# THU-luvision/TextureFusion

Measured on AMD Instinct MI355X. Metric: RGB-D frames/s (TSDF integrate + atlas update: prepare->integrate->finalize, UpdateMeshes, GeneratePatches + UpdateAtlas over the frame's dirty chunks), higher is better.
Workload: dtype f32

## Files before the change

texturefusion_amd/csrc/tf_group.hip:

```cpp
#include <hip/hip_runtime.h>
#include <stdlib.h>

#include <type_traits>

#include "tf_device.h"
#include "tf_devfn.h"
#include "tf_host_math.h"
#include "tf_voxel_math.h"

#pragma clang fp contract(off)

namespace tf {

constexpr int kGroupMax = 6;
struct GroupArgs {
  const float* depth[kGroupMax];
  const float4* pre[kGroupMax];
  const float* cen[kGroupMax];
  int n;
};

struct GroupPoses {
  Pose P[kGroupMax];
};
// ... 83 lines not shown
          __builtin_amdgcn_make_buffer_rsrc((void*)key.img.depth, 0, W * H * 4, 0x00020000);
      const __amdgpu_buffer_rsrc_t rs_rgba =
          __builtin_amdgcn_make_buffer_rsrc((void*)key.img.rgba, 0, W * H * 4, 0x00020000);
      const __amdgpu_buffer_rsrc_t rs_C =
          __builtin_amdgcn_make_buffer_rsrc((void*)(v.color + (size_t)slot * kChunkVoxels), 0, 4096, 0x00020000);
      const __amdgpu_buffer_rsrc_t rs_qual =
          __builtin_amdgcn_make_buffer_rsrc((void*)key.img.quality, 0, QUAL ? W * H * 4 : 0, 0x00020000);
      const float khalf = kc.res * 0.5f;
      const float fx = (float)(lane & 7), fy = (float)vy;
      float qx[3], qy[3];
#pragma unroll
      for (int a = 0; a < 3; ++a) { qx[a] = key.P.p[a] * fx; qy[a] = key.P.p[4 + a] * fy; }
      auto cen = [&](const int a, const int j) -> float {
        const float q2 = key.P.p[8 + a] * (float)j;
        const float s12 = qy[a] + q2;
        const float d = qx[a] + s12;
        return d * kc.res + khalf;
      };
      int off_d[8];
      unsigned long long vm[8];
      uint32_t R = 64, oob_bits = 0;
      int oob_any = 0;
      auto geometry = [&](auto safe_tag) {
        constexpr bool SAFE = decltype(safe_tag)::value;
#pragma unroll
        for (int j = 0; j < 8; ++j) {
          const f32x2 pxy = o01 + (f32x2){cen(0, j), cen(1, j)};
          const float pzv = o2 + cen(2, j);
          f32x2 q;
          if (SAFE) {
            q = div2_by(pxy, recip_refined(pzv));
          } else {
            q.x = pxy.x / pzv;
            q.y = pxy.y / pzv;
          }
          const f32x2 uw = q * fxy + cxy;
          const int X = SAFE ? cvt_rne_hw(uw.x) : cvt_sat_rne(uw.x);
          const int Y = SAFE ? cvt_rne_hw(uw.y) : cvt_sat_rne(uw.y);
          const bool valid = ((unsigned)(X - 1) < (unsigned)(W - 2)) && ((unsigned)(Y - 1) < (unsigned)(H - 2));
          vm[j] = ballot(valid);
          int od = (__mul24(Y, W) + X) * 4;
          asm volatile("" : "+v"(od));
          off_d[j] = valid ? od : kOOB;
          oob_bits |= (((unsigned)X > (unsigned)(W - 1)) || ((unsigned)Y > (unsigned)(H - 1))) ? (1u << j) : 0u;
        }
      };
      if (div_safe) geometry(std::true_type{});
      else geometry(std::false_type{});
      unsigned long long all_valid = ~0ull;
#pragma unroll
      for (int j = 0; j < 8; ++j) all_valid &= vm[j];
      if (all_valid != ~0ull) {
#pragma unroll
        for (int j = 0; j < 8; ++j) {
          if (R == 64u) {
            const unsigned long long dead = nonzero_bytes(vm[j]) ^ 0x0101010101010101ull;
            if (dead) R = (uint32_t)(j * 8) + ((uint32_t)__builtin_ctzll(dead) >> 3);
          }
          const bool live_lane = (uint32_t)(j * 8 + vy) < R;
          oob_any |= (live_lane && ((oob_bits >> j) & 1u)) ? 1 : 0;
          off_d[j] = live_lane ? off_d[j] : kOOB;
        }
      }
      float dep[8];
#pragma unroll
      for (int j = 0; j < 8; ++j)
        dep[j] = __uint_as_float(__builtin_amdgcn_raw_buffer_load_b32(rs_depth, off_d[j], 0, 0));
#pragma unroll
      for (int j = 0; j < 8; ++j) {
        if ((uint32_t)(j * 8) >= R) break;
        const float d = dep[j];
        const float sd = d - (o2 + cen(2, j));
        const bool act = (uint32_t)(j * 8 + vy) < R;
        const bool dv = (d > cam.nearP) && (cam.farP > d);
        const bool inside = (sd > kc.lower) && (upper > sd);
        const bool F = act && dv && inside;
        const float nw = F ? wD : 0.0f;
        const bool rf_l = row_any(ballot(F));
        key_rows_t += (uint32_t)__popcll(ballot(rf_l)) >> 3;
        if (rf_l) {
          const float ts = __uint_as_float(t[j].x), tw = __uint_as_float(t[j].y);
          const float num = ts * tw + sd * nw;
          const float den = (tw + nw) + kc.sigma;
          const float ns = num / den;
          const float nwt = tw + nw;
          const bool keep = nwt > 0.5f;
          t[j].x = __float_as_uint(keep ? ns : 999.0f);
          t[j].y = __float_as_uint(keep ? nwt : 0.0f);
          dirty_rows |= 1u << j;
        }
      }
      uint32_t lanes_c = 0;
      float qsum_rows = 0.0f;
      const bool some_oob = all_valid != ~0ull;
#pragma unroll
      for (int h = 0; h < 2; ++h) {
        int off_c[4], off_i[4];
        unsigned long long any_c = 0ull;
        unsigned long long mo[QUAL ? 4 : 1];
        unsigned long long any_o = 0ull;
        if (QUAL) {
#pragma unroll
          for (int jj = 0; jj < 4; ++jj) {
            const int j = h * 4 + jj;
            mo[jj] = some_oob ? ballot(((uint32_t)(j * 8 + vy) < R) && ((oob_bits >> j) & 1u)) : 0ull;
            any_o |= mo[jj];
          }
        }
#pragma unroll
        for (int jj = 0; jj < 4; ++jj) {
          const int j = h * 4 + jj;
          const float sd = dep[j] - (o2 + cen(2, j));
          const bool upd = (off_d[j] != kOOB) && (fabsf(sd) < kc.thrCol);
          off_i[jj] = upd ? off_d[j] : kOOB;
          const bool ru_l = row_any(ballot(upd));
          const unsigned long long ru = ballot(ru_l);
          off_c[jj] = ru_l ? (j * 64 + lane) * 8 : kOOB;
          lanes_c += (uint32_t)__popcll(ru);
          any_c |= ru;
        }
        if (any_c == 0ull) {
          if (QUAL && any_o) {
#pragma unroll
            for (int jj = 0; jj < 4; ++jj)
              if (mo[jj]) qsum_rows = kc.qoob;
          }
          continue;
        }
        u32x2 c[4];
        uint32_t in[4];
        float qv[QUAL ? 4 : 1];
#pragma unroll
        for (int jj = 0; jj < 4; ++jj) {
          c[jj] = __builtin_amdgcn_raw_buffer_load_b64(rs_C, off_c[jj], 0, 0);
          in[jj] = __builtin_amdgcn_raw_buffer_load_b32(rs_rgba, off_i[jj], 0, 0);
          if (QUAL) qv[jj] = __uint_as_float(__builtin_amdgcn_raw_buffer_load_b32(rs_qual, off_i[jj], 0, 0));
        }
#pragma unroll
        for (int jj = 0; jj < 4; ++jj) {
          const uint32_t p_rg = __builtin_amdgcn_perm(0u, in[jj], 0x0c010c00u);
          const uint32_t p_ba = __builtin_amdgcn_perm(0u, in[jj], 0x0c030c02u);
          const uint32_t w_rg = c[jj].x, w_ba = c[jj].y;
          const u16x2 in_rg = __builtin_bit_cast(u16x2, p_rg), in_ba = __builtin_bit_cast(u16x2, p_ba);
          u16x2 c_rg = __builtin_bit_cast(u16x2, w_rg), c_ba = __builtin_bit_cast(u16x2, w_ba);
          if (FLAG) {
            c_rg += in_rg;
            c_ba += in_ba;
            const bool halve = (int)__builtin_bit_cast(uint32_t, c_ba) >= (121 << 16);
            const u16x2 h_rg = c_rg >> (unsigned short)2, h_ba = c_ba >> (unsigned short)2;
            c_rg = halve ? h_rg : c_rg;
            c_ba = halve ? h_ba : c_ba;
          } else {
            c_rg -= in_rg;
            c_ba -= in_ba;
          }
          c[jj].x = __builtin_bit_cast(uint32_t, c_rg);
          c[jj].y = __builtin_bit_cast(uint32_t, c_ba);
          __builtin_amdgcn_raw_buffer_store_b64(c[jj], rs_C, off_c[jj], 0, 0);
        }
        if (QUAL) {
          const int rowshift = lane & 56;
#pragma unroll
          for (int jj = 0; jj < 4; ++jj) {
            const int j = h * 4 + jj;
            const unsigned long long mu = ballot(off_i[jj] != kOOB);
            if ((mu | mo[jj]) == 0ull) continue;
            float rowsum = 0.0f;
// ... 15 lines not shown
      const float qsum = QUAL ? qsum_rows : ((ballot(oob_any != 0) != 0ull) ? kc.qoob : 0.0f);
      if (lane == 0) {
        L.list_quality[e] = qsum;
        if (obs_kf >= 0 && qsum > 0.0f && key_rows_t != 0u) {
          const uint32_t at = obs_find(v, obs_pack(slot, obs_kf), true);
          if (at != kInvalidSlot) v.obs_q[at] = qsum;
        }
      }
    }
    for (int f = 0; f < ga.n; ++f) {
      const float4 r0 = ga.pre[f][4 * e], r1 = ga.pre[f][4 * e + 1];
      const float o0 = r0.x, o1 = r0.y, o2 = r0.z, pbx = r0.w, pby = r1.x;
      const f32x2 o01 = {o0, o1};
      const float wD = FLAG ? pbx : -pbx;
      const float upper = pby;
      const float band = 32.0f * kc.res;
      const bool div_safe = (fabsf(o2) > band) && (fabsf(o2) < 1048576.0f) && (fabsf(o0) < 1048576.0f) &&
                            (fabsf(o1) < 1048576.0f) && (kc.res > 1e-6f) && (kc.res < 16.0f);
      const __amdgpu_buffer_rsrc_t rs_depth =
          __builtin_amdgcn_make_buffer_rsrc((void*)ga.depth[f], 0, W * H * 4, 0x00020000);
      int off_d[8];
      unsigned long long vm[8];
      uint32_t R = 64;
      auto geometry = [&](auto safe_tag) {
        constexpr bool SAFE = decltype(safe_tag)::value;
#pragma unroll
        for (int j = 0; j < 8; ++j) {
          const int k = j * 64 + lane;
          const f32x2 pxy = o01 + (f32x2){cenT[f][0][k], cenT[f][1][k]};
          const float pzv = o2 + cenT[f][2][k];
          f32x2 q;
          if (SAFE) {
            q = div2_by(pxy, recip_refined(pzv));
          } else {
            q.x = pxy.x / pzv;
            q.y = pxy.y / pzv;
          }
          const f32x2 uw = q * fxy + cxy;
          const int X = SAFE ? cvt_rne_hw(uw.x) : cvt_sat_rne(uw.x);
          const int Y = SAFE ? cvt_rne_hw(uw.y) : cvt_sat_rne(uw.y);
          const bool valid = ((unsigned)(X - 1) < (unsigned)(W - 2)) && ((unsigned)(Y - 1) < (unsigned)(H - 2));
          vm[j] = ballot(valid);
          int od = (__mul24(Y, W) + X) * 4;
          asm volatile("" : "+v"(od));
          off_d[j] = valid ? od : kOOB;
        }
      };
      if (div_safe) geometry(std::true_type{});
      else geometry(std::false_type{});
      unsigned long long all_valid = ~0ull;
#pragma unroll
      for (int j = 0; j < 8; ++j) all_valid &= vm[j];
      if (all_valid != ~0ull) {
#pragma unroll
        for (int j = 0; j < 8; ++j) {
          if (R == 64u) {
            const unsigned long long dead = nonzero_bytes(vm[j]) ^ 0x0101010101010101ull;
            if (dead) R = (uint32_t)(j * 8) + ((uint32_t)__builtin_ctzll(dead) >> 3);
          }
          const bool live_lane = (uint32_t)(j * 8 + vy) < R;
          off_d[j] = live_lane ? off_d[j] : kOOB;
        }
      }
      float dep[8];
#pragma unroll
      for (int j = 0; j < 8; ++j)
        dep[j] = __uint_as_float(__builtin_amdgcn_raw_buffer_load_b32(rs_depth, off_d[j], 0, 0));
#pragma unroll
      for (int j = 0; j < 8; ++j) {
        if ((uint32_t)(j * 8) >= R) break;
        const float d = dep[j];
        const float sd = d - (o2 + cenT[f][2][j * 64 + lane]);
        const bool act = (uint32_t)(j * 8 + vy) < R;
        const bool dv = (d > cam.nearP) && (cam.farP > d);
        const bool inside = (sd > kc.lower) && (upper > sd);
        const bool F = act && dv && inside;
        const float nw = F ? wD : 0.0f;
        const bool rf_l = row_any(ballot(F));
        rows_total += (uint32_t)__popcll(ballot(rf_l)) >> 3;
        if (rf_l) {
          const float ts = __uint_as_float(t[j].x), tw = __uint_as_float(t[j].y);
          const float num = ts * tw + sd * nw;
          const float den = (tw + nw) + kc.sigma;
          const float ns = num / den;
          const float nwt = tw + nw;
          const bool keep = nwt > 0.5f;
          t[j].x = __float_as_uint(keep ? ns : 999.0f);
          t[j].y = __float_as_uint(keep ? nwt : 0.0f);
          dirty_rows |= 1u << j;
        }
      }
    }
    uint32_t word = 0;
#pragma unroll
    for (int j = 0; j < 8; ++j) {
      const bool wr = ((dirty_rows >> j) & 1u) != 0;
      __builtin_amdgcn_raw_buffer_store_b64(t[j], rs_T, wr ? (j * 64 + lane) * 8 : kOOB, 0, 0);
      if (wr) word |= chunk_summary_bits(__uint_as_float(t[j].x), __uint_as_float(t[j].y), (uint32_t)(j * 64 + lane));
    }
    word = wave_or(word);
    if (lane == 0 && word) atomicOr(&v.summ[slot], word);
    const bool updated = (rows_total | key_rows_t) != 0;
    if (updated && lane == 0) {
      L.list_needs[e] = 1;
      if (part_band(v, id.x, id.y, id.z)) mark_touched(v, L.list_ent[e]);
    }
    const uint32_t rows_key = KEY ? (key_rows_c << 8) : (fin ? (uint32_t)L.list_rows[e] : 0u);
    if (lane == 0) L.list_rows[e] = (uint16_t)(rows_total + key_rows_t < 255u ? rows_total + key_rows_t : 255u);
    if (fin) {
      const bool isnew = L.list_new[e] != 0;
      if (updated || L.list_needs[e]) {
        if (lane == 0) {
          v.mark_epoch[slot] = fin_epoch + 1u;
          if (isnew && !part_band(v, id.x, id.y, id.z)) v.hent[L.list_ent[e]].alive = 1u;
        }
        if (claim_par >= 0) claim_dirty7(v, id, slot, L.list_ent[e], lane, claim_stamp, claim_par);
      } else if (isnew) {
        const uint32_t ent = L.list_ent[e];
        if (rows_key >> 8) {
          uint4* c4 = reinterpret_cast<uint4*>(v.color + (size_t)slot * kChunkVoxels);
#pragma unroll
          for (int k = 0; k < 4; ++k) c4[k * 64 + lane] = make_uint4(0, 0, 0, 0);
        }
        if (v.hent[ent].alive) {
          const uint32_t ds = v.summ[slot];
          if (ds != 0u) {
            const uint32_t f999 = __float_as_uint(999.0f);
            uint4* t4 = reinterpret_cast<uint4*>(v.tsdf + (size_t)slot * kChunkVoxels);
#pragma unroll
            for (int k = 0; k < 4; ++k) t4[k * 64 + lane] = make_uint4(f999, 0u, f999, 0u);
          }
          if (lane == 0) {
            v.hent[ent].alive = 0;
            if (ds != 0u) {
              v.summ[slot] = 0u;
              MeshRec* r = &v.mesh_rec[slot];
              if (r->state & kMsInMap) { r->state = 0u; r->nv = 0; r->nt = 0; }
            }
          }
        }
        if (lane == 0) v.erase_epoch[slot] = fin_epoch + 1u;
      }
    }
  }
}


void launch_pre_frames(const VolumeDev& v, const Pose& keyframe, int n, const float* poses12, float4* pre_scratch,
                       float* cen_scratch, const Integ& ig, float res, const Cam& cam, hipStream_t s, int acquire,
                       uint32_t* clear_word) {
  const IntegrateConsts kc = make_integrate_consts(cam.cxi, cam.cyi, res, 1);
  GroupPoses gp = {};
  for (int f = 0; f < n; ++f)
    for (int q = 0; q < 12; ++q) gp.P[f].p[q] = poses12[12 * f + q];
  hipLaunchKernelGGL(k_pre_group, dim3(128, n + 1 + (acquire ? 1 : 0)), dim3(256), 0, s, v, gp, ig, res, kc.resDiag, pre_scratch,
                     cen_scratch, keyframe, 1, acquire, clear_word);
}

void launch_integrate_group(const VolumeDev& v, int n, const float* const* d_depth, const float* poses12, float4* pre_scratch,
                            float* cen_scratch, const Cam& cam, const Integ& ig, float res, int flag, hipStream_t s, bool have_pre,
                            int32_t obs_kf, int fin, uint32_t fin_epoch, int claim_par, uint32_t claim_stamp,
                            const FrameImages* key_img, const Pose* key_pose) {
  IntegrateConsts kc = make_integrate_consts(cam.cxi, cam.cyi, res, flag);
  GroupArgs ga = {};
  GroupPoses gp = {};
  ga.n = n;
  for (int f = 0; f < n; ++f) {
// ... 20 lines not shown
```

texturefusion_amd/csrc/tf_kernels.hip:

```cpp
#include <stdlib.h>

#include <atomic>
#include "tf_device.h"
#include "tf_devfn.h"
#include "tf_host_math.h"
#include "tf_patch_body.h"
#include "tf_voxel_math.h"

#pragma clang fp contract(off)
#ifndef TF_KA_GP
#define TF_KA_GP 2
#endif


namespace tf {

__global__ void k_reset_ctl(FrameCtl* ctl, VolCtl* vctl) {
  if (blockIdx.x == 0 && threadIdx.x == 0) {
    for (int a = 0; a < 3; ++a) {
      ctl->bbox_key[a] = f2key(1e8f);
      ctl->bbox_key[3 + a] = f2key(-1e8f);
      ctl->min_id[a] = ctl->max_id[a] = ctl->dims[a] = 0;
    }
    ctl->n_coarse = 0;
// ... 395 lines not shown
        int4 id;
        id.x = sx + ((step == 4) ? (lane >> 4) : 0);
        id.y = sy + ((step == 4) ? ((lane >> 2) & 3) : 0);
        id.z = sz + ((step == 4) ? (lane & 3) : 0);
        id.w = 0;
        if (pos < v.max_list) L.list_id[pos] = id;
      }
    }
    if (tile == n_tiles - 1u && threadIdx.x == 0) finish(tile_base + agg);
    __syncthreads();
  }
}
void launch_scan(const VolumeDev& v, int step, hipStream_t s) {
  static std::atomic<uint32_t> g_stamp{0};
  uint32_t stamp;
  do { stamp = (g_stamp.fetch_add(1u) + 1u) & 0x3FFFFFFFu; } while (stamp == 0u);
  hipLaunchKernelGGL(k_scan, dim3(256), dim3(256), 0, s, v, step, stamp);
}

__global__ __launch_bounds__(256) void k_acquire(VolumeDev v) {
  const SelBuf& L = v.sel;
  const uint32_t n = L.ctl->n_list;
  for (uint32_t e = blockIdx.x * 256 + threadIdx.x; e < n; e += gridDim.x * 256) {
    const int4 id = L.list_id[e];
    bool is_new = false;
    uint32_t ent = 0;
    const uint32_t slot = chunk_acquire(v, id, &is_new, &ent);
    L.list_slot[e] = slot;
    L.list_ent[e] = ent;
    L.list_new[e] = is_new ? 1 : 0;
    L.list_needs[e] = 0;
  }
}
void launch_acquire(const VolumeDev& v, hipStream_t s) {
  hipLaunchKernelGGL(k_acquire, dim3(512), dim3(256), 0, s, v);
}

__global__ __launch_bounds__(256) void k_pre(VolumeDev v, Pose P, Integ ig, float res, float resDiag, float4* out_pre,
                                             float* out_cen) {
  const SelBuf& L = v.sel;
  float4* pre = out_pre ? out_pre : L.list_pre;
  if (blockIdx.x == 0) centroid_table(P.p, res, out_cen ? out_cen : L.cen);
  const uint32_t n = L.ctl->n_list <= v.max_list ? L.ctl->n_list : 0u;
  for (uint32_t e = blockIdx.x * 256 + threadIdx.x; e < n; e += gridDim.x * 256) {
    const int4 id = L.list_id[e];
    const ChunkPre cp = chunk_pre(id, P.p, ig, res, resDiag);
    pre[4 * e] = make_float4(cp.a.x, cp.a.y, cp.a.z, cp.b.x);
    pre[4 * e + 1] = make_float4(cp.b.y, __int_as_float(id.x), __int_as_float(id.y), __int_as_float(id.z));
  }
}

__global__ __launch_bounds__(256) void k_lookup(VolumeDev v, uint32_t n) {
  const SelBuf& L = v.sel;
  const uint32_t i = blockIdx.x * 256 + threadIdx.x;
  if (i >= n) return;
  const int4 id = L.list_id[i];
  const uint32_t ent = hash_find(v, pack_id(id.x, id.y, id.z));
  uint32_t slot = kInvalidSlot;
  if (ent != kInvalidSlot && v.hent[ent].alive) slot = v.hent[ent].slot;
  if (slot == kInvalidSlot) atomicOr(&v.vctl->status, kStMissing);
  L.list_slot[i] = slot;
  L.list_ent[i] = (ent == kInvalidSlot) ? 0u : ent;
}
void launch_lookup(const VolumeDev& v, uint32_t n, hipStream_t s) {
  if (!n) return;
  hipLaunchKernelGGL(k_lookup, dim3((n + 255) / 256), dim3(256), 0, s, v, n);
}

#ifndef TF_KF_WAVES
#define TF_KF_WAVES 7
#endif
#ifndef TF_KFP_EXTRA
#define TF_KFP_EXTRA 1
#endif
#ifndef TF_KFP_WAVES
#define TF_KFP_WAVES 7
#endif

typedef uint32_t u32x4 __attribute__((ext_vector_type(4)));
typedef const __attribute__((address_space(4))) u32x4* const_u32x4_ptr;
typedef uint32_t u32x8 __attribute__((ext_vector_type(8)));
typedef const __attribute__((address_space(4))) u32x8* const_u32x8_ptr;

template <bool COLOR, bool QUALITY, bool FUSED, bool FLAG, int GP, bool TL = false>
__device__ __forceinline__ void integrate_body(const VolumeDev& v, const FrameImages& img, const Cam& cam,
                                               const IntegrateConsts& kc, const uint32_t epoch,
                                               const uint32_t bid, const uint32_t nb, const int claim_par = -1) {
  const SelBuf& L = v.sel;
  const int lane = threadIdx.x & 63;
  const uint32_t wave = (uint32_t)__builtin_amdgcn_readfirstlane((int)((bid * 256 + threadIdx.x) >> 6));
  const uint32_t nwaves = nb * 4;
  uint32_t n = L.ctl->n_list <= v.max_list ? L.ctl->n_list : 0u;
  uint32_t nf = n;
  if (FUSED) {
    const unsigned long long pk = L.ctl->emit_pack;
    nf = (uint32_t)pk;
    const unsigned long long tot = (pk & 0xFFFFFFFFull) + (pk >> 32);
    n = tot <= (unsigned long long)v.max_list ? (uint32_t)tot : 0u;
    if (!n) nf = 0;
    if (bid == 0 && threadIdx.x == 0) { L.ctl->n_list = n; L.ctl->n_front = nf; }
  }
  const uint32_t n_items = n;
  auto item_pos = [&](const uint32_t e) -> uint32_t { return FUSED ? list_phys(v, e, nf) : e; };
  const int vy = lane >> 3;
  const int W = cam.W, H = cam.H;
  if (FUSED && bid == 0 && threadIdx.x == 0) {
    for (int a = 0; a < 3; ++a) {
      L.ctl->bbox_key[a] = f2key(1e8f);
      L.ctl->bbox_key[3 + a] = f2key(-1e8f);
    }
  }

  const uint32_t e_first = wave, e_step = nwaves;
  u32x8 rec_next;
  {
    const uint32_t e0 = e_first < n_items ? e_first : 0u;
    const uint32_t p0 = n_items ? item_pos(e0) : 0u;
    rec_next = *(const_u32x8_ptr)(unsigned long long)(&L.list_pre[4 * (p0 < v.max_list ? p0 : 0u)]);
  }

  __shared__ float cenT[3][kChunkVoxels];
  {
    const float4* src = reinterpret_cast<const float4*>(L.cen);
    float4* dst = reinterpret_cast<float4*>(&cenT[0][0]);
    for (int i = threadIdx.x; i < 3 * kChunkVoxels / 4; i += 256) dst[i] = src[i];
  }
  __syncthreads();

  const __amdgpu_buffer_rsrc_t rs_depth =
      __builtin_amdgcn_make_buffer_rsrc((void*)img.depth, 0, W * H * 4, 0x00020000);
  const __amdgpu_buffer_rsrc_t rs_rgba =
      __builtin_amdgcn_make_buffer_rsrc((void*)img.rgba, 0, COLOR ? W * H * 4 : 0, 0x00020000);
  const __amdgpu_buffer_rsrc_t rs_qual =
      __builtin_amdgcn_make_buffer_rsrc((void*)img.quality, 0, QUALITY ? W * H * 4 : 0, 0x00020000);

  const uint32_t row_lo = lane < 32 ? (0xFFu << (lane & 24)) : 0u;
  const uint32_t row_hi = lane < 32 ? 0u : (0xFFu << (lane & 24));
  auto row_any = [&](const unsigned long long m) -> bool {
    return ((((uint32_t)m) & row_lo) | (((uint32_t)(m >> 32)) & row_hi)) != 0u;
  };
  auto ballot = [](const bool b) -> unsigned long long { return __builtin_amdgcn_ballot_w64(b); };

  float c_near = cam.nearP, c_far = cam.farP, c_thr = kc.thrCol, c_lower = kc.lower, c_sigma = kc.sigma;
  asm volatile("" : "+v"(c_near), "+v"(c_far), "+v"(c_thr), "+v"(c_lower), "+v"(c_sigma));

  if (TL && (kc.dbg & 8192u) && lane == 0 && wave < (uint32_t)kPhaseWaves)
  {
    v.phase_buf[wave * 16 + 14] = __builtin_amdgcn_s_memrealtime();
    v.phase_buf[wave * 16 + 8] = 0;
    v.phase_buf[wave * 16 + 9] = 0;
  }

  for (uint32_t e = e_first, e_next = e_first + e_step; e < n_items; e = e_next) {
    const uint32_t pe = item_pos(e);
    const u32x8 prw = rec_next;
    {
      e_next = e + e_step;
      const uint32_t en = e_next < n_items ? e_next : e;
      rec_next = *(const_u32x8_ptr)(unsigned long long)(&L.list_pre[4 * item_pos(en)]);
    }
    const int4 id = make_int4((int)prw[5], (int)prw[6], (int)prw[7], 0);
    const bool owned = part_owned(v, id.x, id.y, id.z);
    if (!owned) {
      if (FUSED && lane == 0) {
        L.list_slot[pe] = kInvalidSlot; L.list_ent[pe] = 0; L.list_new[pe] = 0; L.list_needs[pe] = 0;
        L.list_quality[pe] = 0.0f; L.list_rows[pe] = 0;
      }
      continue;
    }
    const unsigned long long key = pack_id(id.x, id.y, id.z);
    const uint32_t i0 = hash_key(key) & v.hmask;
    u32x4 h0 = {0u, 0u, 0u, 0u};
    uint32_t slot = kInvalidSlot;
    if (FUSED) h0 = *(const_u32x4_ptr)(unsigned long long)(&v.hent[i0]);
    else slot = L.list_slot[pe];
    bool is_new = false;
    uint32_t ent = i0;

    const float o0 = __uint_as_float(prw[0]), o1 = __uint_as_float(prw[1]), o2 = __uint_as_float(prw[2]);
    const float pbx = __uint_as_float(prw[3]), pby = __uint_as_float(prw[4]);
    const f32x2 o01 = {o0, o1};
    const f32x2 fxy = {cam.fxi, cam.fyi}, cxy = {kc.cxs, kc.cys};
    const float wD = FLAG ? pbx : -pbx;
    const float upper = pby;
    const float band = 32.0f * kc.res;
    const bool div_safe = (fabsf(o2) > band) && (fabsf(o2) < 1048576.0f) && (fabsf(o0) < 1048576.0f) &&
                          (fabsf(o1) < 1048576.0f) && (kc.res > 1e-6f) && (kc.res < 16.0f);
    if (TL && (kc.dbg & 8192u) && e == e_first && lane == 0 && wave < (uint32_t)kPhaseWaves) {
      asm volatile("" :: "s"(o0), "s"(o1), "s"(o2), "s"(id.x));
      v.phase_buf[wave * 16 + 15] = __builtin_amdgcn_s_memrealtime();
    }

    int off_d[8];
    int oobl[QUALITY ? 8 : 1];
    int oob_any = 0;
    uint32_t R = 64;
    unsigned long long all_valid = ~0ull;
    uint32_t oob_bits = 0;
    auto geometry = [&](auto safe_tag) {
      constexpr bool SAFE = decltype(safe_tag)::value;
#pragma unroll
      for (int j = 0; j < 8; ++j) {
        const int k = j * 64 + lane;
        const f32x2 pxy = o01 + (f32x2){cenT[0][k], cenT[1][k]};
        const float pzv = o2 + cenT[2][k];
        f32x2 q;
        if (SAFE) {
          q = div2_by(pxy, recip_refined(pzv));
        } else {
          q.x = pxy.x / pzv;
          q.y = pxy.y / pzv;
        }
        const f32x2 uw = q * fxy + cxy;
        const int X = SAFE ? cvt_rne_hw(uw.x) : cvt_sat_rne(uw.x);
        const int Y = SAFE ? cvt_rne_hw(uw.y) : cvt_sat_rne(uw.y);
        const bool valid = ((unsigned)(X - 1) < (unsigned)(W - 2)) && ((unsigned)(Y - 1) < (unsigned)(H - 2));
        all_valid &= ballot(valid);
        int od = (__mul24(Y, W) + X) * 4;
        asm volatile("" : "+v"(od));
        off_d[j] = valid ? od : kOOB;
        if (COLOR) oob_bits |= (((unsigned)X > (unsigned)(W - 1)) || ((unsigned)Y > (unsigned)(H - 1))) ? (1u << j) : 0u;
      }
    };
    if (div_safe) geometry(std::true_type{});
    else geometry(std::false_type{});
    if (QUALITY) {
#pragma unroll
      for (int j = 0; j < 8; ++j) oobl[j] = 0;
    }
    if (all_valid != ~0ull) {
#pragma unroll
      for (int j = 0; j < 8; ++j) {
        if (R == 64u) {
          const unsigned long long vmj = ballot(off_d[j] != kOOB);
          const unsigned long long dead = nonzero_bytes(vmj) ^ 0x0101010101010101ull;
          if (dead) R = (uint32_t)(j * 8) + ((uint32_t)__builtin_ctzll(dead) >> 3);
        }
        const bool live_lane = (uint32_t)(j * 8 + vy) < R;
        if (COLOR) {
          const bool oob = live_lane && ((oob_bits >> j) & 1u);
          oob_any |= oob ? 1 : 0;
          if (QUALITY) oobl[j] = oob ? 1 : 0;
        }
        off_d[j] = live_lane ? off_d[j] : kOOB;
      }
    }

    float dep[8];
#pragma unroll
    for (int j = 0; j < 8; ++j)
      dep[j] = __uint_as_float(__builtin_amdgcn_raw_buffer_load_b32(rs_depth, off_d[j], 0, 0));

    bool lazy_revive = false;
    if (FUSED) {
      if ((((unsigned long long)h0.y << 32) | h0.x) == key && h0.z != kInvalidSlot) {
        slot = h0.z;
        is_new = lazy_revive = (h0.w == 0u);
      } else {
        uint32_t s0 = kInvalidSlot, nw = 1, en = 0;
        if (lane == 0) {
          bool bnew = true;
          s0 = chunk_acquire(v, id, &bnew, &en);
          nw = bnew ? 1u : 0u;
        }
        slot = (uint32_t)__builtin_amdgcn_readfirstlane((int)s0);
        is_new = __builtin_amdgcn_readfirstlane((int)nw) != 0;
        ent = (uint32_t)__builtin_amdgcn_readfirstlane((int)en);
      }
    }
    if (slot == kInvalidSlot) {
      if (FUSED && lane == 0) {
        L.list_slot[pe] = kInvalidSlot; L.list_ent[pe] = 0; L.list_new[pe] = 0; L.list_needs[pe] = 0;
        L.list_quality[pe] = 0.0f; L.list_rows[pe] = 0;
      }
      continue;
    }
    const __amdgpu_buffer_rsrc_t rs_T =
        __builtin_amdgcn_make_buffer_rsrc((void*)(v.tsdf + (size_t)slot * kChunkVoxels), 0, 4096, 0x00020000);
    const __amdgpu_buffer_rsrc_t rs_C =
        __builtin_amdgcn_make_buffer_rsrc((void*)(v.color + (size_t)slot * kChunkVoxels), 0, 4096, 0x00020000);

    float qsum = 0.0f;
    uint32_t lanes_t = 0, lanes_c = 0;
    uint32_t sword = 0;
    unsigned long long m_ok = 0, m_pos = 0, m_neg = 0, m_hvy = 0;

#pragma unroll
    for (int p = 0; p < 8 / GP; ++p) {
      const int g0 = p * GP;
      if ((uint32_t)(g0 * 8) >= R) break;
      float nwv[GP], sd[GP];
      int off_t[GP], off_c[GP], off_i[GP];
      unsigned long long any = 0ull;
#pragma unroll
      for (int j = 0; j < GP; ++j) {
        const int gj = g0 + j;
        const int kb = (gj * 64 + lane) * 8;
        const float d = dep[gj];
        const float s = d - (o2 + cenT[2][gj * 64 + lane]);
        sd[j] = s;
        if (COLOR) {
          const bool upd = (off_d[gj] != kOOB) && (fabsf(s) < c_thr);
          off_i[j] = upd ? off_d[gj] : kOOB;
          const bool ru_l = row_any(ballot(upd));
          const unsigned long long ru = ballot(ru_l);
          off_c[j] = ru_l ? kb : kOOB;
          lanes_c += (uint32_t)__popcll(ru);
          any |= ru;
        }
        const bool act = (uint32_t)(gj * 8 + vy) < R;
        const bool dv = (d > c_near) && (c_far > d);
        const bool inside = (s > c_lower) && (upper > s);
        const bool F = act && dv && inside;
        nwv[j] = F ? wD : 0.0f;
        const bool rf_l = row_any(ballot(F));
        const unsigned long long rf = ballot(rf_l);
        off_t[j] = rf_l ? kb : kOOB;
        lanes_t += (uint32_t)__popcll(rf);
        any |= rf;
      }
      const bool rmw = (any != 0ull) || (COLOR && QUALITY);
      u32x2 t[GP], c[GP];
      uint32_t in[GP];
      float qv[GP];
      if (rmw) {
#pragma unroll
        for (int j = 0; j < GP; ++j) t[j] = __builtin_amdgcn_raw_buffer_load_b64(rs_T, off_t[j], 0, 0);
        if (COLOR) {
#pragma unroll
          for (int j = 0; j < GP; ++j) {
            c[j] = __builtin_amdgcn_raw_buffer_load_b64(rs_C, off_c[j], 0, 0);
            in[j] = __builtin_amdgcn_raw_buffer_load_b32(rs_rgba, off_i[j], 0, 0);
            if (QUALITY) qv[j] = __uint_as_float(__builtin_amdgcn_raw_buffer_load_b32(rs_qual, off_i[j], 0, 0));
          }
        }
      }
      if (rmw) {
#pragma unroll
        for (int j = 0; j < GP; ++j) {
          if (COLOR) {
            const uint32_t p_rg = __builtin_amdgcn_perm(0u, in[j], 0x0c010c00u);
            const uint32_t p_ba = __builtin_amdgcn_perm(0u, in[j], 0x0c030c02u);
            const uint32_t w_rg = c[j].x, w_ba = c[j].y;
            const u16x2 in_rg = __builtin_bit_cast(u16x2, p_rg), in_ba = __builtin_bit_cast(u16x2, p_ba);
            u16x2 c_rg = __builtin_bit_cast(u16x2, w_rg), c_ba = __builtin_bit_cast(u16x2, w_ba);
            if (FLAG) {
              c_rg += in_rg;
              c_ba += in_ba;
              const bool halve = (int)__builtin_bit_cast(uint32_t, c_ba) >= (121 << 16);
              const u16x2 h_rg = c_rg >> (unsigned short)2, h_ba = c_ba >> (unsigned short)2;
              c_rg = halve ? h_rg : c_rg;
              c_ba = halve ? h_ba : c_ba;
            } else {
              c_rg -= in_rg;
              c_ba -= in_ba;
            }
            c[j].x = __builtin_bit_cast(uint32_t, c_rg);
            c[j].y = __builtin_bit_cast(uint32_t, c_ba);
          }
          const float ts = __uint_as_float(t[j].x), tw = __uint_as_float(t[j].y);
          const float nw = nwv[j];
          const float num = ts * tw + sd[j] * nw;
          const float den = (tw + nw) + c_sigma;
          const float ns = num / den;
          const float nwt = tw + nw;
          const bool keep = nwt > 0.5f;
          t[j].x = __float_as_uint(keep ? ns : 999.0f);
          t[j].y = __float_as_uint(keep ? nwt : 0.0f);
        }
      }
      if (rmw) {
#pragma unroll
        for (int j = 0; j < GP; ++j) {
          if (COLOR) __builtin_amdgcn_raw_buffer_store_b64(c[j], rs_C, off_c[j], 0, 0);
          __builtin_amdgcn_raw_buffer_store_b64(t[j], rs_T, off_t[j], 0, 0);
          if (!(kc.dbg & kKaCoarseSumm)) {
            const float fs = __uint_as_float(t[j].x), fw = __uint_as_float(t[j].y);
            const unsigned long long b_ok = ballot(!(fs > 1.0f)), b_pos = ballot(fs > 0.0f) & b_ok;
            const unsigned long long b_neg = ballot(fs < 0.0f), b_hvy = ballot(fw > 50.0f);
            m_ok |= b_ok; m_pos |= b_pos; m_neg |= b_neg; m_hvy |= b_hvy;
            if (g0 + j == 0)
              sword = (b_ok ? 0x1000u : 0u) | (b_pos ? 0x2000u : 0u) | (b_neg ? 0x4000u : 0u) | (b_hvy ? 0x8000u : 0u);
          }
        }
      }
      if (COLOR && QUALITY) {
        const int rowshift = lane & 56;
#pragma unroll
        for (int j = 0; j < GP; ++j) {
          const int gj = g0 + j;
          const unsigned long long mu = ballot(off_i[j] != kOOB);
          const unsigned long long mo = ballot(oobl[gj] != 0);
          if ((mu | mo) == 0ull) continue;
          float rowsum = 0.0f;
          if (mu) {
#pragma unroll
            for (int l = 0; l < 8; ++l) rowsum += __shfl(qv[j], rowshift + l);
          }
          const int left = (int)R - gj * 8;
          const int rmax = left < 8 ? left : 8;
          for (int r = 0; r < rmax; ++r) {
            if ((mo >> (8 * r)) & 0xFFull) qsum = kc.qoob;
            if ((mu >> (8 * r)) & 0xFFull)
              qsum += __int_as_float(__builtin_amdgcn_readlane(__float_as_int(rowsum), 8 * r));
          }
        }
      }
    }
    const uint32_t rows_t = lanes_t >> 3, rows_c = COLOR ? (lanes_c >> 3) : 0u;
    const bool updated = rows_t != 0;
    if (updated) {
      if (kc.dbg & kKaCoarseSumm) {
        if (lane == 0) v.summ[slot] = kSummAny;
      } else {
        const unsigned long long mm[4] = {m_ok, m_pos, m_neg, m_hvy};
#pragma unroll
        for (int b = 0; b < 4; ++b)
          sword |= (mm[b] ? (1u << b) : 0u) | ((mm[b] & 0x0101010101010101ull) ? (0x10u << b) : 0u) | ((mm[b] & 0xFFull) ? (0x100u << b) : 0u);
        if (lane == 0 && sword) atomicOr(&v.summ[slot], sword);
      }
    }
    if (TL && (kc.dbg & 8192u) && lane == 0 && wave < (uint32_t)kPhaseWaves) {
      v.phase_buf[wave * 16 + 8] += 1;
      v.phase_buf[wave * 16 + 9] += rows_t + rows_c;
    }
    if (COLOR && !QUALITY) {
      if (ballot(oob_any != 0) != 0ull) qsum = kc.qoob;
    }

    const bool face = part_band(v, id.x, id.y, id.z);
    if (updated && lane == 0 && (face || lazy_revive)) {
      const uint32_t en = FUSED ? ent : L.list_ent[pe];
      if (face) mark_touched(v, en);
      else v.hent[en].alive = 1u;
    }
    if (FUSED) {
      if (updated) {
        if (lane == 0) v.mark_epoch[slot] = epoch + 1u;
        if (claim_par >= 0) {
          claim_dirty7(v, id, slot, ent, lane, epoch + 1u, claim_par);
        }
      } else if (is_new) {
        if (lane == 0) {
          if (!lazy_revive) v.hent[ent].alive = 0;
          v.mark_epoch[(size_t)v.max_chunks + slot] = epoch + 1u;
        }
        if (rows_c) {
          uint4* c4 = reinterpret_cast<uint4*>(v.color + (size_t)slot * kChunkVoxels);
#pragma unroll
          for (int k = 0; k < 4; ++k) c4[k * 64 + lane] = make_uint4(0, 0, 0, 0);
        }
      }
      if (lane == 0) {
        L.list_slot[pe] = slot;
        L.list_needs[pe] = updated ? 1 : 0;
        L.list_rows[pe] = (uint16_t)(rows_t | (rows_c << 8));
      }
    } else if (lane == 0) {
      if (updated) L.list_needs[pe] = 1;
      L.list_quality[pe] = qsum;
      L.list_rows[pe] = (uint16_t)(rows_t | (rows_c << 8));
    }
  }
}

template <bool COLOR, bool QUALITY, bool FLAG>
__global__ __launch_bounds__(256) void k_integrate(VolumeDev v, FrameImages img, Cam cam, IntegrateConsts kc,
                                                   uint32_t epoch) {
  integrate_body<COLOR, QUALITY, false, FLAG, TF_KA_GP>(v, img, cam, kc, epoch, blockIdx.x, gridDim.x);
}

struct FrameLaunch {
  VolumeDev v;
  FrameImages img;
  Pose P;
  IntegrateConsts kc;
  Cam cam;
  Integ ig;
  uint32_t epoch;
  uint32_t n_ka, n_sel, n_bbox;
  uint32_t rot;
  SelBuf sel1;
  const float* depth1;
  SelectConsts sc1;
  FrameCtl* ctl2;
  const float* depth2;
  Pose P2;
  int claim_par;
  uint32_t n_patch;
  int patch_par;
  KfDev kf_patch;
  uint32_t* progress;
  uint32_t progress_val;
};

template <bool COLOR, bool PATCH, bool TL = false>
__global__ __launch_bounds__(256) __attribute__((amdgpu_waves_per_eu(PATCH ? TF_KFP_WAVES : TF_KF_WAVES, PATCH ? TF_KFP_WAVES : TF_KF_WAVES))) void k_frame(FrameLaunch a) {
  const uint32_t total = a.n_ka + a.n_patch + a.n_sel + a.n_bbox;
  const uint32_t b = blockIdx.x + a.rot < total ? blockIdx.x + a.rot : blockIdx.x + a.rot - total;
  const bool timeline = TL && (a.kc.dbg & 4096u) != 0 && a.n_sel > 0 && a.n_bbox > 0;
  const unsigned long long t0 = timeline ? __builtin_amdgcn_s_memrealtime() : 0ull;
  uint32_t role;
  if (b < a.n_ka) {
    role = 0;
    integrate_body<COLOR, false, true, true, TF_KA_GP, TL>(a.v, a.img, a.cam, a.kc, a.epoch, b, a.n_ka, a.claim_par);
  } else if (PATCH && b < a.n_ka + a.n_patch) {
    role = 3;
    patch_body<true, true, true, TL>(a.v, a.cam, a.patch_par, a.kf_patch, b - a.n_ka, a.n_patch);
  } else if (b < a.n_ka + a.n_patch + a.n_sel) {
    role = 1;
    if (!(TL && (a.kc.dbg & 512u))) {
      VolumeDev v1 = a.v;
      v1.sel = a.sel1;
      select_body<true>(a.depth1, a.cam, a.ig, a.sc1, v1, b - a.n_ka - a.n_patch, a.n_sel);
    }
  } else {
    role = 2;
    if (a.progress && b + 1 == total && threadIdx.x == 0)
      __hip_atomic_store(a.progress, a.progress_val, __ATOMIC_RELAXED, __HIP_MEMORY_SCOPE_SYSTEM);
    if (!(TL && (a.kc.dbg & 1024u))) bbox_body(a.depth2, a.cam, a.P2, a.ctl2, b - a.n_ka - a.n_patch - a.n_sel, a.n_bbox);
  }
  if (timeline) {
    const uint32_t gw = (b * 256 + threadIdx.x) >> 6;
    if ((threadIdx.x & 63) == 0 && gw < (uint32_t)kPhaseWaves) {
      a.v.phase_buf[gw * 16 + 10] = t0;
      a.v.phase_buf[gw * 16 + 11] = __builtin_amdgcn_s_memrealtime();
      a.v.phase_buf[gw * 16 + 12] = role + 1;
      a.v.phase_buf[gw * 16 + 13] = (unsigned)__builtin_amdgcn_s_getreg(20 | (0 << 6) | (3 << 11)) & 15u;
    }
  }
}

static int env_int(const char* name, int dflt) {
  const char* e = getenv(name);
  return e ? atoi(e) : dflt;
}
int device_cus() {
  int dev = 0, cus = 256;
  if (hipGetDevice(&dev) == hipSuccess) {
    hipDeviceProp_t p;
    if (hipGetDeviceProperties(&p, dev) == hipSuccess && p.multiProcessorCount > 0) cus = p.multiProcessorCount;
  }
  return cus;
}
static int ka_blocks_default() { return device_cus() * TF_KF_WAVES; }

void launch_integrate(const VolumeDev& v, const FrameImages& img, const Cam& cam, const Integ& ig,
                      const Pose& pose, float res, int flag, bool use_color, bool use_quality,
                      uint32_t epoch, hipStream_t s, bool have_pre) {
  IntegrateConsts kc = make_integrate_consts(cam.cxi, cam.cyi, res, flag);
  if (!have_pre) hipLaunchKernelGGL(k_pre, dim3(256), dim3(256), 0, s, v, pose, ig, res, kc.resDiag, (float4*)nullptr, (float*)nullptr);
  static const int nblocks = ka_blocks_default();
  const dim3 grid(nblocks > 0 ? nblocks : 2048), block(256);
#define TF_LAUNCH_KA(C, Q)                                                                           \
  do {                                                                                               \
    if (flag) hipLaunchKernelGGL((k_integrate<C, Q, true>), grid, block, 0, s, v, img, cam, kc, epoch);  \
    else hipLaunchKernelGGL((k_integrate<C, Q, false>), grid, block, 0, s, v, img, cam, kc, epoch);      \
  } while (0)
  if (use_color && use_quality) TF_LAUNCH_KA(true, true);
  else if (use_color) TF_LAUNCH_KA(true, false);
  else TF_LAUNCH_KA(false, false);
#undef TF_LAUNCH_KA
}

void launch_frame(const VolumeDev& v, const FrameStage* cur, const FrameStage* next,
                  const FrameStage* next2, const PatchStage* patch, const Cam& cam, const Integ& ig, float res, hipStream_t s,
                  uint32_t* progress, uint32_t* progress_seq) {
  const bool with_patch = patch != nullptr && cur != nullptr && cur->img.rgba != nullptr;
  static const int nblocks7 = ka_blocks_default();
  static const int nblocksP = device_cus() * (TF_KFP_WAVES + TF_KFP_EXTRA);
  const int nblocks = with_patch ? nblocksP : nblocks7;
  FrameLaunch a;
  a.v = v;
  a.cam = cam;
  a.ig = ig;
  a.n_ka = a.n_sel = a.n_bbox = a.n_patch = 0;
  a.patch_par = 0;
  a.claim_par = -1;
  a.epoch = 0;
  a.progress = nullptr;
  a.progress_val = 0;
  if (with_patch) {
    a.n_patch = 1024u;
    a.patch_par = patch->par;
    a.kf_patch = patch->kf;
  }
  a.kc = make_integrate_consts(cam.cxi, cam.cyi, res, 1);
  static const int dbg = env_int("TF_KA_DBG", 0);
  a.kc.dbg = (uint32_t)dbg;
  bool color = false;
  if (cur) {
    a.v.sel = cur->sel;
    a.img = cur->img;
    a.P = cur->pose;
    a.epoch = cur->epoch;
    a.n_ka = (uint32_t)(nblocks > 0 ? nblocks : 2048);
    color = cur->img.rgba != nullptr;
    a.claim_par = cur->claim_par;
    if (cur->coarse_summ) a.kc.dbg |= kKaCoarseSumm;
  }
  if (next) {
    a.sel1 = next->sel;
    a.depth1 = next->img.depth;
    a.sc1 = make_select_consts(next->pose.p, res);
    a.n_sel = 1u;
  }
  if (next2) {
    a.ctl2 = next2->sel.ctl;
    a.depth2 = next2->img.depth;
    a.P2 = next2->pose;
    int nvec = (cam.W * cam.H) >> 2;
    int blocks = (nvec + 255) / 256;
    a.n_bbox = (uint32_t)(blocks > 128 ? 128 : blocks);
  }
  const bool others_first = with_patch && cur->small_frame;
  if (a.n_sel) a.n_sel = others_first ? 128u : 256u;
  const uint32_t total = a.n_ka + a.n_patch + a.n_sel + a.n_bbox;
  if (!total) return;
  if (progress && progress_seq && a.n_bbox) {
    a.progress = progress;
    a.progress_val = ++*progress_seq;
  }
  if ((a.kc.dbg & 4096u) && a.n_sel && a.n_bbox) a.kc.dbg |= 8192u;
  a.rot = others_first ? a.n_ka : 0u;
  const bool tuning = dbg != 0 || (with_patch && a.kf_patch.pad[0] != 0);
  if (with_patch) {
    if (tuning) hipLaunchKernelGGL((k_frame<true, true, true>), dim3(total), dim3(256), 0, s, a);
    else hipLaunchKernelGGL((k_frame<true, true>), dim3(total), dim3(256), 0, s, a);
  } else if (color) {
    if (tuning) hipLaunchKernelGGL((k_frame<true, false, true>), dim3(total), dim3(256), 0, s, a);
    else hipLaunchKernelGGL((k_frame<true, false>), dim3(total), dim3(256), 0, s, a);
  } else {
    hipLaunchKernelGGL((k_frame<false, false>), dim3(total), dim3(256), 0, s, a);
  }
}

__global__ __launch_bounds__(256) void k_finalize(VolumeDev v, uint32_t epoch) {
  const SelBuf& L = v.sel;
  const uint32_t n = L.ctl->n_list;
  const int sub = threadIdx.x & 7;
  __shared__ uint32_t dead[32], dsumm[32];
  __shared__ uint32_t ndead;
  for (uint32_t base = blockIdx.x * 32; base < n; base += gridDim.x * 32) {
    if (threadIdx.x == 0) ndead = 0;
    __syncthreads();
    const uint32_t e = base + (threadIdx.x >> 3);
    if (e < n) {
      const int4 id = L.list_id[e];
      const bool owned = part_owned(v, id.x, id.y, id.z);
      const bool needs = L.list_needs[e] != 0;
      const bool isnew = L.list_new[e] != 0;
      if (owned && needs && sub == 0) {
        const uint32_t slot = L.list_slot[e];
        if (slot != kInvalidSlot) v.mark_epoch[slot] = epoch + 1u;
      }
      if (owned && sub == 7 && !needs && isnew) {
        const uint32_t slot = L.list_slot[e];
        const uint32_t ent = L.list_ent[e];
        if (slot != kInvalidSlot && v.hent[ent].alive) {
          v.hent[ent].alive = 0;
          const uint32_t di = atomicAdd(&ndead, 1u);
          dead[di] = slot;
          dsumm[di] = v.summ[slot];
        }
        if (slot != kInvalidSlot) v.erase_epoch[slot] = epoch + 1u;
      }
    }
    __syncthreads();
    const uint32_t nd = ndead;
    for (uint32_t k = 0; k < nd; ++k) {
      const uint32_t ds = dead[k];
      uint4* c4 = reinterpret_cast<uint4*>(v.color + (size_t)ds * kChunkVoxels);
      c4[threadIdx.x] = make_uint4(0, 0, 0, 0);
      if (dsumm[k] != 0u) {
        const uint32_t f999 = __float_as_uint(999.0f);
        uint4* t4 = reinterpret_cast<uint4*>(v.tsdf + (size_t)ds * kChunkVoxels);
        t4[threadIdx.x] = make_uint4(f999, 0u, f999, 0u);
      }
    }
    if (threadIdx.x < nd && dsumm[threadIdx.x] != 0u) {
      const uint32_t ds = dead[threadIdx.x];
      {
// ... 325 lines not shown
```

texturefusion_amd/csrc/tf_voxel_math.h:

```cpp
#pragma once

#include "tf_devfn.h"
#include "tf_device.h"
#include "tf_host_math.h"

#pragma clang fp contract(off)

namespace tf {

__device__ __forceinline__ int cvt_rne(float x) {
  return (x >= -2147483648.0f && x < 2147483648.0f) ? (int)rintf(x) : (int)0x80000000;
}

__device__ __forceinline__ uint32_t f2key(float f) {
  uint32_t b = __float_as_uint(f);
  return (b & 0x80000000u) ? ~b : (b | 0x80000000u);
}
__device__ __forceinline__ float key2f(uint32_t k) {
  uint32_t b = (k & 0x80000000u) ? (k & 0x7FFFFFFFu) : ~k;
  return __uint_as_float(b);
}

__device__ __forceinline__ float truncation(const Integ& ig, float z) {
  double zz = (double)z * (double)z;
// ... 24 lines not shown
  r.a = make_float4(o[0], o[1], o[2], trunc);
  r.b = make_float4(ig.weight / (2.0f * trunc), trunc + resDiag, 0.0f, 0.0f);
  return r;
}


__device__ __forceinline__ void centroid_table(const float* __restrict__ Pp, float res, float* __restrict__ cen) {
  const float half = res * 0.5f;
  for (int i = threadIdx.x; i < kChunkVoxels; i += 256) {
    const float fx = (float)(i & 7), fy = (float)((i >> 3) & 7), fz = (float)(i >> 6);
#pragma unroll
    for (int a = 0; a < 3; ++a) {
      const float q0 = Pp[a] * fx, q1 = Pp[4 + a] * fy, q2 = Pp[8 + a] * fz;
      const float s12 = q1 + q2;
      const float d = q0 + s12;
      cen[a * kChunkVoxels + i] = d * res + half;
    }
  }
}


__device__ __forceinline__ void acquire_emitted_body(const VolumeDev& v, const uint32_t bid, const uint32_t nb, const bool lazy = false) {
  const SelBuf& L = v.sel;
  const unsigned long long pk = L.ctl->emit_pack;
  uint32_t n = (uint32_t)pk;
  if ((pk >> 32) != 0ull || n > v.max_list) n = 0;
  if (bid == 0 && threadIdx.x == 0) {
    L.ctl->n_list = n;
    L.ctl->n_front = n;
    for (int a = 0; a < 3; ++a) { L.ctl->bbox_key[a] = f2key(1e8f); L.ctl->bbox_key[3 + a] = f2key(-1e8f); }
  }
  for (uint32_t e = bid * 256 + threadIdx.x; e < n; e += nb * 256) {
    const int4 id = L.list_id[e];
    bool is_new = false;
    uint32_t ent = 0;
    const uint32_t slot = chunk_acquire(v, id, &is_new, &ent, lazy);
    L.list_slot[e] = slot;
    L.list_ent[e] = ent;
    L.list_new[e] = is_new ? 1 : 0;
    L.list_needs[e] = 0;
  }
}

__device__ __forceinline__ unsigned long long nonzero_bytes(unsigned long long m) {
  unsigned long long t = m | (m >> 1);
  t |= t >> 2;
  t |= t >> 4;
  return t & 0x0101010101010101ull;
}

typedef unsigned int u32x2 __attribute__((ext_vector_type(2)));
constexpr int kOOB = 0x7FFFFFF0;


__device__ __forceinline__ int cvt_sat_rne(float x) {
  return (int)rintf(__builtin_amdgcn_fmed3f(x, -2147483648.0f, 2147483520.0f));
}

__device__ __forceinline__ int cvt_rne_hw(float x) {
  int r;
  const float n = rintf(x);
  asm("v_cvt_i32_f32_e32 %0, %1" : "=v"(r) : "v"(n));
  return r;
}

struct Recip { float d, r; };
__device__ __forceinline__ Recip recip_refined(float d) {
  Recip R;
  R.d = d;
  const float r0 = __builtin_amdgcn_rcpf(d);
  const float e = __builtin_fmaf(-d, r0, 1.0f);
  R.r = __builtin_fmaf(e, r0, r0);
  return R;
}
typedef float f32x2 __attribute__((ext_vector_type(2)));
__device__ __forceinline__ f32x2 div2_by(const f32x2 n, const Recip& R) {
  const f32x2 d = {-R.d, -R.d}, r = {R.r, R.r};
  const f32x2 q0 = n * r;
  const f32x2 e0 = __builtin_elementwise_fma(d, q0, n);
  const f32x2 q1 = __builtin_elementwise_fma(e0, r, q0);
  const f32x2 e1 = __builtin_elementwise_fma(d, q1, n);
  return __builtin_elementwise_fma(e1, r, q1);
}

typedef unsigned short u16x2 __attribute__((ext_vector_type(2)));

__device__ __forceinline__ void claim_dirty7(const VolumeDev& v, const int4 id, const uint32_t slot, const uint32_t ent, const int lane,
                                             const uint32_t stamp, const int par) {
  uint32_t cs = kInvalidSlot, ce = 0;
  int4 q = id;
  if (lane < 7) {
    q = nbr7(id, lane);
    if (lane == 0) { cs = slot; ce = ent; }
    else if (part_owned(v, q.x, q.y, q.z)) cs = hash_slot_alive_ent(v, pack_id(q.x, q.y, q.z), &ce);
    if (cs != kInvalidSlot && !(atomicMax(&v.mesh_rec[cs].stamp, stamp) < stamp)) cs = kInvalidSlot;
    if (cs != kInvalidSlot) {
      const uint32_t rows = v.max_chunks / kMeshShards + 258u;
      const uint32_t sh = cs & (kMeshShards - 1u);
      const uint32_t p = atomicAdd(&v.wl_cnt[((par & 1) * kMeshShards + sh) * 16], 1u);
      if (p < rows) {
        const size_t at = ((size_t)(par & 1) * kMeshShards + sh) * rows + p;
        v.wl_ids[at] = make_int4(q.x, q.y, q.z, (int)(ce + 1u));
        v.wl_slot[at] = cs;
      } else {
        atomicOr(&v.vctl->status, kStMeshFull);
      }
    }
  }
}

__device__ __forceinline__ unsigned long long obs_pack(uint32_t slot, int32_t kf) {
  return ((unsigned long long)slot << 32) | (unsigned long long)(uint32_t)kf;
}
__device__ __forceinline__ uint32_t obs_find(const VolumeDev& v, unsigned long long key, bool insert) {
  uint32_t i = hash_key(key) & v.obs_mask;
  for (uint32_t probe = 0; probe <= v.obs_mask; ++probe) {
    unsigned long long cur = v.obs_key[i];
    if (cur == kEmptyKey) {
      if (!insert) return kInvalidSlot;
      cur = atomicCAS(&v.obs_key[i], kEmptyKey, key);
      if (cur == kEmptyKey) return i;
    }
    if (cur == key) return i;
    i = (i + 1) & v.obs_mask;
  }
  if (insert) atomicOr(&v.vctl->status, kStHashFull);
  return kInvalidSlot;
}

}
```

Baseline: 10690.

## Reload integrate args from kernarg, fast exact divide, per-lane summary class bits

The integrate body now reads its volume, image, camera and constants through an accessor that can fetch them straight from the kernarg segment inside the loop, and builds buffer resources at their point of use. This shortens live ranges and is meant to cut SGPR/VGPR pressure. The TSDF divide becomes a wave-uniform fast path (reciprocal plus Newton refinement) when all lanes' operands are in a safe magnitude range, with IEEE division as the fallback. The per-row summary ballots are replaced by per-lane class bits that are reduced once per chunk. Coarse summaries are disabled when patches are fused into the same launch, which adds some extra summary work on that path.

```diff
diff --git a/texturefusion_amd/csrc/tf_group.hip b/texturefusion_amd/csrc/tf_group.hip
--- a/texturefusion_amd/csrc/tf_group.hip
+++ b/texturefusion_amd/csrc/tf_group.hip
@@ -189,7 +189,7 @@
           const float ts = __uint_as_float(t[j].x), tw = __uint_as_float(t[j].y);
           const float num = ts * tw + sd * nw;
           const float den = (tw + nw) + kc.sigma;
-          const float ns = num / den;
+          const float ns = div_exact(num, den);
           const float nwt = tw + nw;
           const bool keep = nwt > 0.5f;
           t[j].x = __float_as_uint(keep ? ns : 999.0f);
@@ -371,7 +371,7 @@
           const float ts = __uint_as_float(t[j].x), tw = __uint_as_float(t[j].y);
           const float num = ts * tw + sd * nw;
           const float den = (tw + nw) + kc.sigma;
-          const float ns = num / den;
+          const float ns = div_exact(num, den);
           const float nwt = tw + nw;
           const bool keep = nwt > 0.5f;
           t[j].x = __float_as_uint(keep ? ns : 999.0f);
diff --git a/texturefusion_amd/csrc/tf_kernels.hip b/texturefusion_amd/csrc/tf_kernels.hip
--- a/texturefusion_amd/csrc/tf_kernels.hip
+++ b/texturefusion_amd/csrc/tf_kernels.hip
@@ -501,10 +501,35 @@
 typedef uint32_t u32x8 __attribute__((ext_vector_type(8)));
 typedef const __attribute__((address_space(4))) u32x8* const_u32x8_ptr;
 
-template <bool COLOR, bool QUALITY, bool FUSED, bool FLAG, int GP, bool TL = false>
-__device__ __forceinline__ void integrate_body(const VolumeDev& v, const FrameImages& img, const Cam& cam,
-                                               const IntegrateConsts& kc, const uint32_t epoch,
+struct KaArgs {
+  const VolumeDev& v_;
+  const FrameImages& img_;
+  const Cam& cam_;
+  const IntegrateConsts& kc_;
+  __device__ const VolumeDev& v() const { return v_; }
+  __device__ const FrameImages& img() const { return img_; }
+  __device__ const Cam& cam() const { return cam_; }
+  __device__ const IntegrateConsts& kc() const { return kc_; }
+};
+template <class FL>
+struct KaArgsFrame {
+  __device__ static const __attribute__((address_space(4))) FL* rec() {
+    const __attribute__((address_space(4))) FL* q = (const __attribute__((address_space(4))) FL*)__builtin_amdgcn_kernarg_segment_ptr();
+    asm volatile("" : "+s"(q));
+    return q;
+  }
+  __device__ const VolumeDev& v() const { return *(const VolumeDev*)&rec()->v; }
+  __device__ const FrameImages& img() const { return *(const FrameImages*)&rec()->img; }
+  __device__ const Cam& cam() const { return *(const Cam*)&rec()->cam; }
+  __device__ const IntegrateConsts& kc() const { return *(const IntegrateConsts*)&rec()->kc; }
+};
+
+template <bool COLOR, bool QUALITY, bool FUSED, bool FLAG, int GP, bool TL = false, bool COARSE = true, class ARGS>
+__device__ __forceinline__ void integrate_body(const ARGS& A, const uint32_t epoch,
                                                const uint32_t bid, const uint32_t nb, const int claim_par = -1) {
+  const VolumeDev& v = A.v();
+  const Cam& cam = A.cam();
+  const IntegrateConsts& kc = A.kc();
   const SelBuf& L = v.sel;
   const int lane = threadIdx.x & 63;
   const uint32_t wave = (uint32_t)__builtin_amdgcn_readfirstlane((int)((bid * 256 + threadIdx.x) >> 6));
@@ -546,13 +571,6 @@
   }
   __syncthreads();
 
-  const __amdgpu_buffer_rsrc_t rs_depth =
-      __builtin_amdgcn_make_buffer_rsrc((void*)img.depth, 0, W * H * 4, 0x00020000);
-  const __amdgpu_buffer_rsrc_t rs_rgba =
-      __builtin_amdgcn_make_buffer_rsrc((void*)img.rgba, 0, COLOR ? W * H * 4 : 0, 0x00020000);
-  const __amdgpu_buffer_rsrc_t rs_qual =
-      __builtin_amdgcn_make_buffer_rsrc((void*)img.quality, 0, QUALITY ? W * H * 4 : 0, 0x00020000);
-
   const uint32_t row_lo = lane < 32 ? (0xFFu << (lane & 24)) : 0u;
   const uint32_t row_hi = lane < 32 ? 0u : (0xFFu << (lane & 24));
   auto row_any = [&](const unsigned long long m) -> bool {
@@ -571,6 +589,12 @@
   }
 
   for (uint32_t e = e_first, e_next = e_first + e_step; e < n_items; e = e_next) {
+    const VolumeDev& v = A.v();
+    const SelBuf& L = v.sel;
+    const FrameImages& img = A.img();
+    const Cam& cam = A.cam();
+    const IntegrateConsts& kc = A.kc();
+    const int W = cam.W, H = cam.H;
     const uint32_t pe = item_pos(e);
     const u32x8 prw = rec_next;
     {
@@ -665,6 +689,8 @@
       }
     }
 
+    const __amdgpu_buffer_rsrc_t rs_depth =
+        __builtin_amdgcn_make_buffer_rsrc((void*)img.depth, 0, W * H * 4, 0x00020000);
     float dep[8];
 #pragma unroll
     for (int j = 0; j < 8; ++j)
@@ -701,8 +727,7 @@
 
     float qsum = 0.0f;
     uint32_t lanes_t = 0, lanes_c = 0;
-    uint32_t sword = 0;
-    unsigned long long m_ok = 0, m_pos = 0, m_neg = 0, m_hvy = 0;
+    uint32_t cls = 0;
 
 #pragma unroll
     for (int p = 0; p < 8 / GP; ++p) {
@@ -746,6 +771,10 @@
 #pragma unroll
         for (int j = 0; j < GP; ++j) t[j] = __builtin_amdgcn_raw_buffer_load_b64(rs_T, off_t[j], 0, 0);
         if (COLOR) {
+          const __amdgpu_buffer_rsrc_t rs_rgba =
+              __builtin_amdgcn_make_buffer_rsrc((void*)img.rgba, 0, COLOR ? W * H * 4 : 0, 0x00020000);
+          const __amdgpu_buffer_rsrc_t rs_qual =
+              __builtin_amdgcn_make_buffer_rsrc((void*)img.quality, 0, QUALITY ? W * H * 4 : 0, 0x00020000);
 #pragma unroll
           for (int j = 0; j < GP; ++j) {
             c[j] = __builtin_amdgcn_raw_buffer_load_b64(rs_C, off_c[j], 0, 0);
@@ -755,6 +784,12 @@
         }
       }
       if (rmw) {
+        float ns[GP];
+#pragma unroll
+        for (int j = 0; j < GP; ++j) {
+          const float ts = __uint_as_float(t[j].x), tw = __uint_as_float(t[j].y);
+          ns[j] = div_exact(ts * tw + sd[j] * nwv[j], (tw + nwv[j]) + c_sigma);
+        }
 #pragma unroll
         for (int j = 0; j < GP; ++j) {
           if (COLOR) {
@@ -777,14 +812,9 @@
             c[j].x = __builtin_bit_cast(uint32_t, c_rg);
             c[j].y = __builtin_bit_cast(uint32_t, c_ba);
           }
-          const float ts = __uint_as_float(t[j].x), tw = __uint_as_float(t[j].y);
-          const float nw = nwv[j];
-          const float num = ts * tw + sd[j] * nw;
-          const float den = (tw + nw) + c_sigma;
-          const float ns = num / den;
-          const float nwt = tw + nw;
+          const float nwt = __uint_as_float(t[j].y) + nwv[j];
           const bool keep = nwt > 0.5f;
-          t[j].x = __float_as_uint(keep ? ns : 999.0f);
+          t[j].x = __float_as_uint(keep ? ns[j] : 999.0f);
           t[j].y = __float_as_uint(keep ? nwt : 0.0f);
         }
       }
@@ -793,13 +823,11 @@
         for (int j = 0; j < GP; ++j) {
           if (COLOR) __builtin_amdgcn_raw_buffer_store_b64(c[j], rs_C, off_c[j], 0, 0);
           __builtin_amdgcn_raw_buffer_store_b64(t[j], rs_T, off_t[j], 0, 0);
-          if (!(kc.dbg & kKaCoarseSumm)) {
+          if (!(COARSE && (kc.dbg & kKaCoarseSumm))) {
             const float fs = __uint_as_float(t[j].x), fw = __uint_as_float(t[j].y);
-            const unsigned long long b_ok = ballot(!(fs > 1.0f)), b_pos = ballot(fs > 0.0f) & b_ok;
-            const unsigned long long b_neg = ballot(fs < 0.0f), b_hvy = ballot(fw > 50.0f);
-            m_ok |= b_ok; m_pos |= b_pos; m_neg |= b_neg; m_hvy |= b_hvy;
-            if (g0 + j == 0)
-              sword = (b_ok ? 0x1000u : 0u) | (b_pos ? 0x2000u : 0u) | (b_neg ? 0x4000u : 0u) | (b_hvy ? 0x8000u : 0u);
+            const bool ok = !(fs > 1.0f);
+            const uint32_t cj = (ok ? 1u : 0u) | ((ok && fs > 0.0f) ? 2u : 0u) | ((fs < 0.0f) ? 4u : 0u) | ((fw > 50.0f) ? 8u : 0u);
+            cls |= (g0 + j == 0) ? (cj | (cj << 4)) : cj;
           }
         }
       }
@@ -829,13 +857,16 @@
     const uint32_t rows_t = lanes_t >> 3, rows_c = COLOR ? (lanes_c >> 3) : 0u;
     const bool updated = rows_t != 0;
     if (updated) {
-      if (kc.dbg & kKaCoarseSumm) {
+      if (COARSE && (kc.dbg & kKaCoarseSumm)) {
         if (lane == 0) v.summ[slot] = kSummAny;
       } else {
-        const unsigned long long mm[4] = {m_ok, m_pos, m_neg, m_hvy};
-#pragma unroll
-        for (int b = 0; b < 4; ++b)
-          sword |= (mm[b] ? (1u << b) : 0u) | ((mm[b] & 0x0101010101010101ull) ? (0x10u << b) : 0u) | ((mm[b] & 0xFFull) ? (0x100u << b) : 0u);
+        uint32_t sword = 0;
+#pragma unroll
+        for (int b = 0; b < 4; ++b) {
+          const unsigned long long mm = ballot((cls >> b) & 1u), m0 = ballot((cls >> (4 + b)) & 1u);
+          sword |= (mm ? (1u << b) : 0u) | ((mm & 0x0101010101010101ull) ? (0x10u << b) : 0u) | ((mm & 0xFFull) ? (0x100u << b) : 0u) |
+                   (m0 ? (0x1000u << b) : 0u);
+        }
         if (lane == 0 && sword) atomicOr(&v.summ[slot], sword);
       }
     }
@@ -886,7 +917,7 @@
 template <bool COLOR, bool QUALITY, bool FLAG>
 __global__ __launch_bounds__(256) void k_integrate(VolumeDev v, FrameImages img, Cam cam, IntegrateConsts kc,
                                                    uint32_t epoch) {
-  integrate_body<COLOR, QUALITY, false, FLAG, TF_KA_GP>(v, img, cam, kc, epoch, blockIdx.x, gridDim.x);
+  integrate_body<COLOR, QUALITY, false, FLAG, TF_KA_GP>(KaArgs{v, img, cam, kc}, epoch, blockIdx.x, gridDim.x);
 }
 
 struct FrameLaunch {
@@ -922,7 +953,7 @@
   uint32_t role;
   if (b < a.n_ka) {
     role = 0;
-    integrate_body<COLOR, false, true, true, TF_KA_GP, TL>(a.v, a.img, a.cam, a.kc, a.epoch, b, a.n_ka, a.claim_par);
+    integrate_body<COLOR, false, true, true, TF_KA_GP, TL, !PATCH || TL>(KaArgsFrame<FrameLaunch>{}, a.epoch, b, a.n_ka, a.claim_par);
   } else if (PATCH && b < a.n_ka + a.n_patch) {
     role = 3;
     patch_body<true, true, true, TL>(a.v, a.cam, a.patch_par, a.kf_patch, b - a.n_ka, a.n_patch);
@@ -1016,7 +1047,7 @@
     a.n_ka = (uint32_t)(nblocks > 0 ? nblocks : 2048);
     color = cur->img.rgba != nullptr;
     a.claim_par = cur->claim_par;
-    if (cur->coarse_summ) a.kc.dbg |= kKaCoarseSumm;
+    if (cur->coarse_summ && !with_patch) a.kc.dbg |= kKaCoarseSumm;
   }
   if (next) {
     a.sel1 = next->sel;
diff --git a/texturefusion_amd/csrc/tf_voxel_math.h b/texturefusion_amd/csrc/tf_voxel_math.h
--- a/texturefusion_amd/csrc/tf_voxel_math.h
+++ b/texturefusion_amd/csrc/tf_voxel_math.h
@@ -130,6 +130,23 @@
   const f32x2 e1 = __builtin_elementwise_fma(d, q1, n);
   return __builtin_elementwise_fma(e1, r, q1);
 }
+__device__ __forceinline__ float div1_by(const float n, const Recip& R) {
+  const float q0 = n * R.r;
+  const float e0 = __builtin_fmaf(-R.d, q0, n);
+  const float q1 = __builtin_fmaf(e0, R.r, q0);
+  const float e1 = __builtin_fmaf(-R.d, q1, n);
+  return __builtin_fmaf(e1, R.r, q1);
+}
+__device__ __forceinline__ bool mag_2p40(const float x) {
+  return (__float_as_uint(x) & 0x7FFFFFFFu) - 0x2B800000u <= 0x28000000u;
+}
+__device__ __forceinline__ bool div_plain(const float n, const float d) {
+  return mag_2p40(d) && (mag_2p40(n) || __float_as_uint(n) == 0u);
+}
+__device__ __forceinline__ float div_exact(const float n, const float d) {
+  if (__builtin_amdgcn_ballot_w64(!div_plain(n, d)) == 0ull) return div1_by(n, recip_refined(d));
+  return n / d;
+}
 
 typedef unsigned short u16x2 __attribute__((ext_vector_type(2)));
 
```

Result: no change. 10480, median of 2 (-2.0%).
